# SFR-Vision/6d-pose-estimation

Measured on NVIDIA B200. Metric: ADD-S pose evals/sec (2k-pt mesh), higher is better.
Workload: dtype f32

## Files before the change

### 6d-pose-estimation_b200/csrc/p6d_adds_pruned.cu

```cuda
#include <algorithm>
#include <atomic>
#include <map>
#include <memory>
#include <mutex>
#include <vector>

#include "p6d_common.cuh"

namespace p6d {

constexpr int PR_BLOCK = 32;
constexpr int PR_SUB = 8;
constexpr float PR_SENTINEL = 1.0e18f;
constexpr int PR_MIN_POINTS = 128;

struct PrunedSlot {
    int64_t offset;
    int32_t nb;
    int32_t floats;
};
__host__ __device__ inline int pr_floats(int nb) {
    const int np = PR_BLOCK * nb, nbp = (nb + 3) / 4 * 4;
    return 3 * np + 3 * nbp + 12 * nb + np / 2;
}

struct PrunedTable {
    float* d_sorted = nullptr;
    PrunedSlot* d_slots = nullptr;
    std::vector<PrunedSlot> h_slots;
    int max_nb = 0;
    int max_count = 0;
    std::atomic<bool> enabled{false};
};

static std::mutex g_pr_mu;
static std::map<const p6d_mesh_table*, PrunedTable*> g_pr_tables;

static void kd_split(const float* xyz, std::vector<int>& idx, int lo, int hi) {
    if (hi - lo <= PR_SUB) return;
    const int unit = hi - lo > PR_BLOCK ? PR_BLOCK : PR_SUB;
    float mn[3] = {1e30f, 1e30f, 1e30f}, mx[3] = {-1e30f, -1e30f, -1e30f};
    for (int i = lo; i < hi; ++i)
        for (int c = 0; c < 3; ++c) {
            const float v = xyz[3 * idx[i] + c];
            if (v < mn[c]) mn[c] = v;
            if (v > mx[c]) mx[c] = v;
        }
    int axis = 0;
    for (int c = 1; c < 3; ++c)
        if (mx[c] - mn[c] > mx[axis] - mn[axis]) axis = c;
    const int blocks = (hi - lo + unit - 1) / unit;
    const int mid = lo + (blocks + 1) / 2 * unit;
    auto key = [&](int i) { const float v = xyz[3 * i + axis]; return v == v ? v : 3.0e38f; };
    std::nth_element(idx.begin() + lo, idx.begin() + mid, idx.begin() + hi, [&](int a, int b) {
        const float va = key(a), vb = key(b);
        return va < vb || (va == vb && a < b);
    });
    kd_split(xyz, idx, lo, mid);
    kd_split(xyz, idx, mid, hi);
}

static PrunedTable* build_pruned(const p6d_mesh_table* t, const float* xyz, const int32_t* offsets) {
    std::unique_ptr<PrunedTable> pt(new PrunedTable());
    pt->h_slots.resize(t->n_slots);
    size_t total = 0;
    for (int s = 0; s < t->n_slots; ++s) {
        const int n = t->h_slots[s].count;
        PrunedSlot& ps = pt->h_slots[s];
        ps.nb = (n + PR_BLOCK - 1) / PR_BLOCK;
        ps.floats = pr_floats(ps.nb);
        ps.offset = static_cast<int64_t>(total);
        total += static_cast<size_t>(ps.floats);
        pt->max_nb = std::max(pt->max_nb, ps.nb);
        pt->max_count = std::max(pt->max_count, n);
    }
    std::vector<float> buf(total > 0 ? total : 4, 0.0f);
    for (int s = 0; s < t->n_slots; ++s) {
        const int n = t->h_slots[s].count;
        if (n == 0) continue;
        const PrunedSlot& ps = pt->h_slots[s];
        const float* src = xyz + 3 * static_cast<size_t>(offsets[s]);
        std::vector<int> idx(n);
        for (int i = 0; i < n; ++i) idx[i] = i;
        kd_split(src, idx, 0, n);
        const int np = PR_BLOCK * ps.nb, nbp = (ps.nb + 3) / 4 * 4;
        float* x = buf.data() + ps.offset;
        float* cen = x + 3 * np;
        float* sub = cen + 3 * nbp;
        const int ns = 4 * ps.nb;
        uint16_t* perm = reinterpret_cast<uint16_t*>(sub + 3 * ns);
        for (int b = 0; b < ps.nb; ++b) {
            double c[3] = {0.0, 0.0, 0.0};
            const int cnt = std::min(PR_BLOCK, n - PR_BLOCK * b);
            for (int l = 0; l < PR_BLOCK; ++l) {
                const int p = PR_BLOCK * b + l;
                const int i = idx[l < cnt ? p : PR_BLOCK * b];
                for (int k = 0; k < 3; ++k) x[k * np + p] = src[3 * i + k];
                perm[p] = l < cnt ? static_cast<uint16_t>(i) : 0xffffu;
                if (l < cnt)
                    for (int k = 0; k < 3; ++k) c[k] += src[3 * i + k];
            }
            for (int k = 0; k < 3; ++k) cen[k * nbp + b] = static_cast<float>(c[k] / cnt);
            for (int q = 0; q < PR_BLOCK / PR_SUB; ++q) {
                double sc[3] = {0.0, 0.0, 0.0};
                const int first = PR_BLOCK * b + PR_SUB * q;
                const int scnt = std::max(0, std::min(PR_SUB, n - first));
                for (int l = 0; l < scnt; ++l)
                    for (int k = 0; k < 3; ++k) sc[k] += x[k * np + first + l];
                for (int k = 0; k < 3; ++k)
                    sub[k * ns + 4 * b + q] = scnt > 0 ? static_cast<float>(sc[k] / scnt) : x[k * np + PR_BLOCK * b];
            }
        }
    }
    if (cudaMalloc(&pt->d_sorted, buf.size() * sizeof(float)) != cudaSuccess ||
        cudaMalloc(&pt->d_slots, t->n_slots * sizeof(PrunedSlot)) != cudaSuccess ||
        cudaMemcpy(pt->d_sorted, buf.data(), buf.size() * sizeof(float), cudaMemcpyHostToDevice) != cudaSuccess ||
        cudaMemcpy(pt->d_slots, pt->h_slots.data(), t->n_slots * sizeof(PrunedSlot), cudaMemcpyHostToDevice) !=
            cudaSuccess) {
        cudaGetLastError();
        if (pt->d_sorted) cudaFree(pt->d_sorted);
        if (pt->d_slots) cudaFree(pt->d_slots);
        return nullptr;
    }
    return pt.release();
}

void pruned_table_release(const p6d_mesh_table* t) {
    PrunedTable* pt = nullptr;
    {
        std::lock_guard<std::mutex> lock(g_pr_mu);
        auto it = g_pr_tables.find(t);
        if (it == g_pr_tables.end()) return;
        pt = it->second;
        g_pr_tables.erase(it);
    }
    cudaFree(pt->d_sorted);
    cudaFree(pt->d_slots);
    delete pt;
}

struct PrunedArgs {
    const float* sorted;
    const PrunedSlot* pslots;
};

__host__ __device__ inline size_t pr_smem_floats(int nb, int nmax) {
    const int np = PR_BLOCK * nb;
    return static_cast<size_t>(pr_floats(nb)) + 3 * np + 3 * np + 2 * static_cast<size_t>((nmax + 3) / 4 * 4) + 4 * nb + 16 * nb;
}

__device__ __forceinline__ float eval_block(const float4* __restrict__ q, float px, float py, float pz, float m) {
    float m2 = __int_as_float(0x7f800000);
#pragma unroll
    for (int k = 0; k < PR_BLOCK / 4; ++k) {
        const float4 X = q[3 * k], Y = q[3 * k + 1], Z = q[3 * k + 2];
        const float2 pxx = make_float2(px, px), pyy = make_float2(py, py), pzz = make_float2(pz, pz);
        {
            const float2 dx = sub2(pxx, make_float2(X.x, X.y)), dy = sub2(pyy, make_float2(Y.x, Y.y)),
                         dz = sub2(pzz, make_float2(Z.x, Z.y));
            const float2 s = fma2(dz, dz, fma2(dy, dy, mul2(dx, dx)));
            m = min3_nan(m, s.x, s.y);
        }
        {
            const float2 dx = sub2(pxx, make_float2(X.z, X.w)), dy = sub2(pyy, make_float2(Y.z, Y.w)),
                         dz = sub2(pzz, make_float2(Z.z, Z.w));
            const float2 s = fma2(dz, dz, fma2(dy, dy, mul2(dx, dx)));
            m2 = min3_nan(m2, s.x, s.y);
        }
    }
    return min_nan(m, m2);
}

__device__ __forceinline__ float eval_sub(const float4* __restrict__ q, float px, float py, float pz, float m) {
    const float2 pxx = make_float2(px, px), pyy = make_float2(py, py), pzz = make_float2(pz, pz);
    float m2 = __int_as_float(0x7f800000);
#pragma unroll
    for (int k = 0; k < PR_SUB / 4; ++k) {
        const float4 X = q[3 * k], Y = q[3 * k + 1], Z = q[3 * k + 2];
        {
            const float2 dx = sub2(pxx, make_float2(X.x, X.y)), dy = sub2(pyy, make_float2(Y.x, Y.y)),
                         dz = sub2(pzz, make_float2(Z.x, Z.y));
            const float2 s = fma2(dz, dz, fma2(dy, dy, mul2(dx, dx)));
            m = min3_nan(m, s.x, s.y);
        }
        {
            const float2 dx = sub2(pxx, make_float2(X.z, X.w)), dy = sub2(pyy, make_float2(Y.z, Y.w)),
                         dz = sub2(pzz, make_float2(Z.z, Z.w));
            const float2 s = fma2(dz, dz, fma2(dy, dy, mul2(dx, dx)));
            m2 = min3_nan(m2, s.x, s.y);
        }
    }
    return min_nan(m, m2);
}

__device__ __forceinline__ float eval_two(const float4* __restrict__ q0, const float4* __restrict__ q1, float px, float py,
                                          float pz, float m) {
    const float a = eval_sub(q0, px, py, pz, m);
    const float b = eval_sub(q1, px, py, pz, __int_as_float(0x7f800000));
    return min_nan(a, b);
}

template <int T, int MINB>
__global__ void __launch_bounds__(T, MINB) adds_pruned_kernel(EvalArgs a, PrunedArgs pa, int nb_max, int nmax) {
    constexpr int PR_WARPS = T / 32;
    extern __shared__ __align__(128) unsigned char smem_raw[];
    const int np_max = PR_BLOCK * nb_max;
    float* s_sorted = reinterpret_cast<float*>(smem_raw);
    float* s_gt = s_sorted + pr_floats(nb_max);
    float* s_pred = s_gt + 3 * np_max;
    float* s_dadd = s_pred + 3 * np_max;
    float* s_dadds = s_dadd + (nmax + 3) / 4 * 4;
    float4* s_cp = reinterpret_cast<float4*>(s_dadds + (nmax + 3) / 4 * 4);
    float4* s_cg = s_cp + nb_max;
    __shared__ uint64_t s_bar;
    __shared__ float s_pose[14];
    __shared__ float s_mean[2];
    __shared__ long long s_oid;
    __shared__ int s_next;
    __shared__ int s_blk[2];

    const unsigned full = 0xffffffffu;
    const int tid = threadIdx.x, lane = tid & 31, warp = tid >> 5;
    if (tid == 0) {
        mbar_init(&s_bar, 1);
        fence_mbar_init();
        s_blk[0] = PR_WARPS;
        s_blk[1] = PR_WARPS;
    }
    int par = 0;
    long long staged_oid = -1;
    uint32_t phase = 0;
    if (tid == 0) s_next = atomicAdd(a.work_counter, 1);
    __syncthreads();

    for (;;) {
        const int64_t it = s_next;
        if (it >= a.B) break;
        const int64_t b = a.order ? a.order[it] : it;
        if (tid < 4) s_pose[tid] = __ldg(a.pq + 4 * b + tid);
        else if (tid < 8) s_pose[tid] = __ldg(a.gq + 4 * b + tid - 4);
        else if (tid < 11) s_pose[tid] = __ldg(a.pt + 3 * b + tid - 8);
        else if (tid < 14) s_pose[tid] = __ldg(a.gt + 3 * b + tid - 11);
        else if (tid == 32) s_oid = a.obj[b];
        __syncthreads();
        if (tid == 64) s_next = atomicAdd(a.work_counter, 1);
        const long long oid = s_oid;
        const bool known = oid >= 0 && oid < a.n_slots && a.slots[oid].count > 0;
        if (!known) {
            if (tid == 0) {
                a.add[b] = 0.0f;
                a.adds[b] = 0.0f;
                a.hit[b] = 0;
                a.valid[b] = 0;
                if (a.borderline) a.borderline[b] = 0;
            }
            __syncthreads();
            continue;
        }
        const SlotInfo s = a.slots[oid];
        const PrunedSlot ps = pa.pslots[oid];
        const int n = s.count, nb = ps.nb, np = PR_BLOCK * nb, nbp = (nb + 3) / 4 * 4;
        if (oid != staged_oid) {
            if (tid == 0) {
                fence_proxy_async();
                const uint32_t bytes = static_cast<uint32_t>(ps.floats) * sizeof(float);
                mbar_arrive_expect_tx(&s_bar, bytes);
                tma_bulk_g2s(s_sorted, pa.sorted + ps.offset, bytes, &s_bar);
            }
            mbar_wait(&s_bar, phase);
            phase ^= 1;
            staged_oid = oid;
        }
        const float* mx = s_sorted;
        const float* my = mx + np;
        const float* mz = my + np;
        const float* cen = mz + np;
        const float* sub = cen + 3 * nbp;
        const int ns = 4 * nb;
        const uint16_t* perm = reinterpret_cast<const uint16_t*>(sub + 3 * ns);
        const int mode = s.xform_mode;

        {
            float Rp[9], Rg[9], tp[3], tg[3];
            quat_to_mat(s_pose, Rp);
            quat_to_mat(s_pose + 4, Rg);
#pragma unroll
            for (int k = 0; k < 3; ++k) {
                tp[k] = s_pose[8 + k];
                tg[k] = s_pose[11 + k];
            }
            for (int blk = warp; blk < nb; blk += PR_WARPS) {
                const int p = PR_BLOCK * blk + lane;
                const unsigned orig = perm[p];
                const bool valid = orig != 0xffffu;
                const float x = mx[p], y = my[p], z = mz[p];
                float px, py, pz, qx, qy, qz;
                xform_point(mode, x, y, z, Rp, tp, px, py, pz);
                xform_point(mode, x, y, z, Rg, tg, qx, qy, qz);
                s_pred[p] = px;
                s_pred[np + p] = py;
                s_pred[2 * np + p] = pz;
                float* gq = s_gt + (p >> 2) * 12 + (p & 3);
                gq[0] = valid ? qx : PR_SENTINEL;
                gq[4] = valid ? qy : PR_SENTINEL;
                gq[8] = valid ? qz : PR_SENTINEL;
                if (valid) s_dadd[orig] = __fsqrt_rn(sq3(__fsub_rn(px, qx), __fsub_rn(py, qy), __fsub_rn(pz, qz)));
                const float cx = cen[blk], cy = cen[nbp + blk], cz = cen[2 * nbp + blk];
                const int sb = 4 * blk + (lane >> 3);
                const float sx = sub[sb], sy = sub[ns + sb], sz = sub[2 * ns + sb];
                float cpx, cpy, cpz, cgx, cgy, cgz;
                xform_point(XF_FMA_CHAIN, cx, cy, cz, Rp, tp, cpx, cpy, cpz);
                xform_point(XF_FMA_CHAIN, sx, sy, sz, Rg, tg, cgx, cgy, cgz);
                const float dp = sqrtf(sq3(px - cpx, py - cpy, pz - cpz));
                const float dg = sqrtf(sq3(qx - cgx, qy - cgy, qz - cgz));
                const unsigned rp = __reduce_max_sync(full, valid ? __float_as_uint(dp) : 0u);
                unsigned rg = valid ? __float_as_uint(dg) : 0u;
                rg = max(rg, __shfl_xor_sync(full, rg, 1));
                rg = max(rg, __shfl_xor_sync(full, rg, 2));
                rg = max(rg, __shfl_xor_sync(full, rg, 4));
                if (lane == 0) s_cp[blk] = make_float4(cpx, cpy, cpz, __uint_as_float(rp) * 1.00001f);
                if ((lane & 7) == 0) s_cg[sb] = make_float4(cgx, cgy, cgz, __uint_as_float(rg) * 1.00001f);
            }
        }
        __syncthreads();

        {
            const float4* gq4 = reinterpret_cast<const float4*>(s_gt);
            int A = warp;
            while (A < nb) {
                const int p = PR_BLOCK * A + lane;
                const unsigned orig = perm[p];
                const bool valid = orig != 0xffffu;
                const float px = s_pred[p], py = s_pred[np + p], pz = s_pred[2 * np + p];
                float m = eval_block(gq4 + 24 * A, px, py, pz, __int_as_float(0x7f800000));
                const float4 cA = s_cp[A];
                for (int c0 = 0; c0 < ns; c0 += 32) {
                    const float mmax = __uint_as_float(__reduce_max_sync(full, valid ? __float_as_uint(m) : 0u));
                    const float th = sqrtf(mmax) * 1.0001f + cA.w;
                    const int Bq = c0 + lane;
                    bool cand = false;
                    if (Bq < ns && (Bq >> 2) != A) {
                        const float4 cB = s_cg[Bq];
                        const float dx = cA.x - cB.x, dy = cA.y - cB.y, dz = cA.z - cB.z;
                        const float d2 = dx * dx + dy * dy + dz * dz;
                        const float rhs = th + cB.w;
                        const bool skip = d2 * 0.9999f >= rhs * rhs && d2 < 3.0e38f;
                        cand = !skip;
                    }
                    unsigned todo = __ballot_sync(full, cand);
                    while (todo) {
                        const int b0 = __ffs(todo) - 1;
                        todo &= todo - 1;
                        if (todo) {
                            const int b1 = __ffs(todo) - 1;
                            todo &= todo - 1;
                            m = eval_two(gq4 + 6 * (c0 + b0), gq4 + 6 * (c0 + b1), px, py, pz, m);
                        } else {
                            m = eval_sub(gq4 + 6 * (c0 + b0), px, py, pz, m);
                        }
                    }
                }
                if (valid) s_dadds[orig] = __fsqrt_rn(m);
                int nxt = 0;
                if (lane == 0) nxt = atomicAdd(&s_blk[par], 1);
                A = __shfl_sync(full, nxt, 0);
            }
        }
        __syncthreads();
        if (tid == 0) s_blk[par] = PR_WARPS;
        par ^= 1;

        if (tid < 64) {
            const float* src = tid < 32 ? s_dadd : s_dadds;
            const float mean = aten_mean_warp([&](int e) { return src[e]; }, n, lane);
            if (lane == 0) s_mean[tid >> 5] = mean;
            asm volatile("bar.sync 1, 64;" ::: "memory");
            if (tid == 0) {
                const float add = s_mean[0], adds = s_mean[1];
                const float eff = s.symmetric ? adds : add;
                const bool is_hit = static_cast<double>(eff) < s.threshold;
                a.add[b] = add;
                a.adds[b] = adds;
                a.hit[b] = is_hit ? 1 : 0;
                a.valid[b] = 1;
                if (a.borderline) a.borderline[b] = near_threshold(eff, s.threshold) ? 1 : 0;
                accumulate(a, oid, is_hit, add, adds, true);
            }
        }
    }
}

static size_t g_pr_smem_raised[64];

int launch_eval_pruned(const p6d_mesh_table* table, const EvalArgs& args, cudaStream_t st, bool force, bool* used) {
    *used = false;
    PrunedTable* ptab = nullptr;
    {
        std::lock_guard<std::mutex> lock(g_pr_mu);
        auto it = g_pr_tables.find(table);
        if (it != g_pr_tables.end()) ptab = it->second;
    }
    if (!ptab || (!force && (!ptab->enabled.load(std::memory_order_relaxed) || table->max_count < PR_MIN_POINTS))) return P6D_OK;
    const int nb = ptab->max_nb > 0 ? ptab->max_nb : 1;
    const size_t smem = sizeof(float) * pr_smem_floats(nb, table->max_count);
    {
        std::lock_guard<std::mutex> lock(g_pr_mu);
        size_t& cur = g_pr_smem_raised[table->device & 63];
        if (smem > cur) {
            int limit = 0;
            P6D_CUDA(cudaDeviceGetAttribute(&limit, cudaDevAttrMaxSharedMemoryPerBlockOptin, table->device));
            if (smem + 1024 > static_cast<size_t>(limit)) {
                if (!force) return P6D_OK;
                set_error("largest mesh has %d points; the pruned ADD-S kernel keeps both clouds and the sorted mesh in "
                          "shared memory and accepts at most %d points on this device (p6d_add_eval takes larger meshes)",
                          table->max_count, (limit - 1024) / 4 / 12 / 32 * 32);
                return P6D_ETOOBIG;
            }
            for (const void* fn : {(const void*)adds_pruned_kernel<256, 2>, (const void*)adds_pruned_kernel<256, 3>,
                                   (const void*)adds_pruned_kernel<256, 4>, (const void*)adds_pruned_kernel<128, 8>})
                P6D_CUDA(cudaFuncSetAttribute(fn, cudaFuncAttributeMaxDynamicSharedMemorySize, static_cast<int>(smem)));
            cur = smem;
        }
    }
    EvalArgs a = args;
    a.work_counter = table->d_counters + (__atomic_fetch_add(&table->counter_idx, 1u, __ATOMIC_RELAXED) % P6D_NUM_COUNTERS);
    P6D_CUDA(cudaMemsetAsync(a.work_counter, 0, sizeof(int), st));
    struct Shape { const void* fn; int threads, minb; };
    const Shape shapes[] = {{(const void*)adds_pruned_kernel<128, 8>, 128, 8}, {(const void*)adds_pruned_kernel<256, 4>, 256, 4},
                            {(const void*)adds_pruned_kernel<256, 3>, 256, 3}, {(const void*)adds_pruned_kernel<256, 2>, 256, 2}};
    const Shape* pick = &shapes[3];
    int per_sm = 0;
    for (const Shape& sh : shapes) {
        if (sh.threads == 128 && nb > 16) continue;
        int occ = 0;
        P6D_CUDA(cudaOccupancyMaxActiveBlocksPerMultiprocessor(&occ, sh.fn, sh.threads, smem));
        if (occ >= sh.minb || &sh == &shapes[3]) {
            pick = &sh;
            per_sm = occ;
            break;
        }
    }
    if (per_sm < 1) per_sm = 1;
    int64_t grid = static_cast<int64_t>(table->sm_count) * per_sm;
    if (grid > a.B) grid = a.B;
    PrunedArgs pa{ptab->d_sorted, ptab->d_slots};
    int nb_arg = nb, nmax_arg = table->max_count;
    void* kargs[] = {&a, &pa, &nb_arg, &nmax_arg};
    P6D_CUDA(cudaLaunchKernel(pick->fn, dim3(static_cast<unsigned>(grid)), dim3(pick->threads), kargs, smem, st));
    P6D_CUDA(cudaGetLastError());
    *used = true;
    return P6D_OK;
}

}

using namespace p6d;

extern "C" {

void p6d_internal_build_pruned(const p6d_mesh_table* t, const float* xyz, const int32_t* offsets) {
    if (t->max_count > 65534) return;
    PrunedTable* pt = nullptr;
    try {
        pt = build_pruned(t, xyz, offsets);
    } catch (...) {
        return;
    }
    if (!pt) return;
    std::lock_guard<std::mutex> lock(g_pr_mu);
    g_pr_tables[t] = pt;
}

void p6d_internal_release_pruned(const p6d_mesh_table* t) { pruned_table_release(t); }

int p6d_mesh_table_set_pruning(p6d_mesh_table* table, int enable) {
    if (!table) { set_error("p6d_mesh_table_set_pruning: table is NULL"); return P6D_EINVAL; }
    std::lock_guard<std::mutex> lock(g_pr_mu);
    auto it = g_pr_tables.find(table);
    if (it == g_pr_tables.end()) {
        if (!enable) return P6D_OK;
        set_error("p6d_mesh_table_set_pruning: this table has no block structure (a mesh with more than 65,534 points, "
                  "or out of memory at creation)");
        return P6D_ETOOBIG;
    }
    it->second->enabled.store(enable != 0, std::memory_order_relaxed);
    return P6D_OK;
}

int p6d_add_eval_pruned(const p6d_mesh_table* table, const float* pq, const float* pt, const float* gq,
                        const float* gt, const int64_t* obj, const int32_t* order, int64_t B, float* add,
                        float* adds, uint8_t* hit, uint8_t* valid, uint8_t* borderline,
                        const p6d_accumulators* acc, void* stream) {
    if (!table || B < 0 || (B > 0 && (!pq || !pt || !gq || !gt || !obj || !add || !adds || !hit || !valid))) {
        set_error("p6d_add_eval_pruned: bad arguments");
        return P6D_EINVAL;
    }
    auto mis = [](const void* p, size_t al) { return p && (reinterpret_cast<uintptr_t>(p) & (al - 1)) != 0; };
    if (mis(pq, 4) || mis(pt, 4) || mis(gq, 4) || mis(gt, 4) || mis(obj, 8) || mis(order, 4) || mis(add, 4) || mis(adds, 4)) {
        set_error("p6d_add_eval_pruned: a pointer is not aligned to its element size");
        return P6D_EINVAL;
    }
    if (B == 0) return P6D_OK;
    if (B > static_cast<int64_t>(INT32_MAX) - (1 << 20)) {
        set_error("p6d_add_eval_pruned: B = %lld exceeds the per-launch limit of %d poses; split the batch",
                  static_cast<long long>(B), INT32_MAX - (1 << 20));
        return P6D_EINVAL;
    }
    DeviceGuard guard(table->device);
    if (!guard.ok) return cuda_fail(cudaGetLastError(), "cudaSetDevice");
    EvalArgs a{};
    fill_eval_args(table, a);
    a.pq = pq; a.pt = pt; a.gq = gq; a.gt = gt; a.obj = obj; a.order = order; a.B = B;
    a.add = add; a.adds = adds; a.hit = hit; a.valid = valid; a.borderline = borderline;
    if (acc) { a.acc = *acc; a.has_acc = 1; }
    bool used = false;
    const int rc = launch_eval_pruned(table, a, static_cast<cudaStream_t>(stream), true, &used);
    if (rc == P6D_OK && !used) {
        set_error("p6d_add_eval_pruned: this table has no block structure (a mesh with more than 65,534 points, or out of "
                  "memory at creation)");
        return P6D_ETOOBIG;
    }
    return rc;
}

}
```

Before: 1.386 million.

## Read sorted mesh from global, drop pred smem, prune with per-sub-block spheres

```diff
diff --git a/6d-pose-estimation_b200/csrc/p6d_adds_pruned.cu b/6d-pose-estimation_b200/csrc/p6d_adds_pruned.cu
--- a/6d-pose-estimation_b200/csrc/p6d_adds_pruned.cu
+++ b/6d-pose-estimation_b200/csrc/p6d_adds_pruned.cu
@@ -19,9 +19,9 @@
     int32_t nb;
     int32_t floats;
 };
-__host__ __device__ inline int pr_floats(int nb) {
-    const int np = PR_BLOCK * nb, nbp = (nb + 3) / 4 * 4;
-    return 3 * np + 3 * nbp + 12 * nb + np / 2;
+inline int pr_floats(int nb) {
+    const int np = PR_BLOCK * nb;
+    return 3 * np + 12 * nb + np / 2;
 }
 
 struct PrunedTable {
@@ -83,24 +83,19 @@
         std::vector<int> idx(n);
         for (int i = 0; i < n; ++i) idx[i] = i;
         kd_split(src, idx, 0, n);
-        const int np = PR_BLOCK * ps.nb, nbp = (ps.nb + 3) / 4 * 4;
+        const int np = PR_BLOCK * ps.nb;
         float* x = buf.data() + ps.offset;
-        float* cen = x + 3 * np;
-        float* sub = cen + 3 * nbp;
+        float* sub = x + 3 * np;
         const int ns = 4 * ps.nb;
         uint16_t* perm = reinterpret_cast<uint16_t*>(sub + 3 * ns);
         for (int b = 0; b < ps.nb; ++b) {
-            double c[3] = {0.0, 0.0, 0.0};
             const int cnt = std::min(PR_BLOCK, n - PR_BLOCK * b);
             for (int l = 0; l < PR_BLOCK; ++l) {
                 const int p = PR_BLOCK * b + l;
                 const int i = idx[l < cnt ? p : PR_BLOCK * b];
                 for (int k = 0; k < 3; ++k) x[k * np + p] = src[3 * i + k];
                 perm[p] = l < cnt ? static_cast<uint16_t>(i) : 0xffffu;
-                if (l < cnt)
-                    for (int k = 0; k < 3; ++k) c[k] += src[3 * i + k];
-            }
-            for (int k = 0; k < 3; ++k) cen[k * nbp + b] = static_cast<float>(c[k] / cnt);
+            }
             for (int q = 0; q < PR_BLOCK / PR_SUB; ++q) {
                 double sc[3] = {0.0, 0.0, 0.0};
                 const int first = PR_BLOCK * b + PR_SUB * q;
@@ -146,7 +141,7 @@
 
 __host__ __device__ inline size_t pr_smem_floats(int nb, int nmax) {
     const int np = PR_BLOCK * nb;
-    return static_cast<size_t>(pr_floats(nb)) + 3 * np + 3 * np + 2 * static_cast<size_t>((nmax + 3) / 4 * 4) + 4 * nb + 16 * nb;
+    return 3 * static_cast<size_t>(np) + 2 * static_cast<size_t>((nmax + 3) / 4 * 4) + 32 * static_cast<size_t>(nb);
 }
 
 __device__ __forceinline__ float eval_block(const float4* __restrict__ q, float px, float py, float pz, float m) {
@@ -200,19 +195,20 @@
     return min_nan(a, b);
 }
 
+#ifdef P6D_DEV
+__device__ unsigned long long g_pr_sub_evals;
+#endif
+
 template <int T, int MINB>
 __global__ void __launch_bounds__(T, MINB) adds_pruned_kernel(EvalArgs a, PrunedArgs pa, int nb_max, int nmax) {
     constexpr int PR_WARPS = T / 32;
     extern __shared__ __align__(128) unsigned char smem_raw[];
     const int np_max = PR_BLOCK * nb_max;
-    float* s_sorted = reinterpret_cast<float*>(smem_raw);
-    float* s_gt = s_sorted + pr_floats(nb_max);
-    float* s_pred = s_gt + 3 * np_max;
-    float* s_dadd = s_pred + 3 * np_max;
+    float4* s_cp = reinterpret_cast<float4*>(smem_raw);
+    float4* s_cg = s_cp + 4 * nb_max;
+    float* s_gt = reinterpret_cast<float*>(s_cg + 4 * nb_max);
+    float* s_dadd = s_gt + 3 * np_max;
     float* s_dadds = s_dadd + (nmax + 3) / 4 * 4;
-    float4* s_cp = reinterpret_cast<float4*>(s_dadds + (nmax + 3) / 4 * 4);
-    float4* s_cg = s_cp + nb_max;
-    __shared__ uint64_t s_bar;
     __shared__ float s_pose[14];
     __shared__ float s_mean[2];
     __shared__ long long s_oid;
@@ -222,14 +218,10 @@
     const unsigned full = 0xffffffffu;
     const int tid = threadIdx.x, lane = tid & 31, warp = tid >> 5;
     if (tid == 0) {
-        mbar_init(&s_bar, 1);
-        fence_mbar_init();
         s_blk[0] = PR_WARPS;
         s_blk[1] = PR_WARPS;
     }
     int par = 0;
-    long long staged_oid = -1;
-    uint32_t phase = 0;
     if (tid == 0) s_next = atomicAdd(a.work_counter, 1);
     __syncthreads();
 
@@ -259,24 +251,11 @@
         }
         const SlotInfo s = a.slots[oid];
         const PrunedSlot ps = pa.pslots[oid];
-        const int n = s.count, nb = ps.nb, np = PR_BLOCK * nb, nbp = (nb + 3) / 4 * 4;
-        if (oid != staged_oid) {
-            if (tid == 0) {
-                fence_proxy_async();
-                const uint32_t bytes = static_cast<uint32_t>(ps.floats) * sizeof(float);
-                mbar_arrive_expect_tx(&s_bar, bytes);
-                tma_bulk_g2s(s_sorted, pa.sorted + ps.offset, bytes, &s_bar);
-            }
-            mbar_wait(&s_bar, phase);
-            phase ^= 1;
-            staged_oid = oid;
-        }
-        const float* mx = s_sorted;
+        const int n = s.count, nb = ps.nb, np = PR_BLOCK * nb, ns = 4 * nb;
+        const float* mx = pa.sorted + ps.offset;
         const float* my = mx + np;
         const float* mz = my + np;
-        const float* cen = mz + np;
-        const float* sub = cen + 3 * nbp;
-        const int ns = 4 * nb;
+        const float* sub = mz + np;
         const uint16_t* perm = reinterpret_cast<const uint16_t*>(sub + 3 * ns);
         const int mode = s.xform_mode;
 
@@ -291,63 +270,88 @@
             }
             for (int blk = warp; blk < nb; blk += PR_WARPS) {
                 const int p = PR_BLOCK * blk + lane;
-                const unsigned orig = perm[p];
+                const unsigned orig = __ldg(perm + p);
                 const bool valid = orig != 0xffffu;
-                const float x = mx[p], y = my[p], z = mz[p];
+                const float x = __ldg(mx + p), y = __ldg(my + p), z = __ldg(mz + p);
                 float px, py, pz, qx, qy, qz;
                 xform_point(mode, x, y, z, Rp, tp, px, py, pz);
                 xform_point(mode, x, y, z, Rg, tg, qx, qy, qz);
-                s_pred[p] = px;
-                s_pred[np + p] = py;
-                s_pred[2 * np + p] = pz;
                 float* gq = s_gt + (p >> 2) * 12 + (p & 3);
                 gq[0] = valid ? qx : PR_SENTINEL;
                 gq[4] = valid ? qy : PR_SENTINEL;
                 gq[8] = valid ? qz : PR_SENTINEL;
                 if (valid) s_dadd[orig] = __fsqrt_rn(sq3(__fsub_rn(px, qx), __fsub_rn(py, qy), __fsub_rn(pz, qz)));
-                const float cx = cen[blk], cy = cen[nbp + blk], cz = cen[2 * nbp + blk];
                 const int sb = 4 * blk + (lane >> 3);
-                const float sx = sub[sb], sy = sub[ns + sb], sz = sub[2 * ns + sb];
+                const float sx = __ldg(sub + sb), sy = __ldg(sub + ns + sb), sz = __ldg(sub + 2 * ns + sb);
                 float cpx, cpy, cpz, cgx, cgy, cgz;
-                xform_point(XF_FMA_CHAIN, cx, cy, cz, Rp, tp, cpx, cpy, cpz);
+                xform_point(XF_FMA_CHAIN, sx, sy, sz, Rp, tp, cpx, cpy, cpz);
                 xform_point(XF_FMA_CHAIN, sx, sy, sz, Rg, tg, cgx, cgy, cgz);
                 const float dp = sqrtf(sq3(px - cpx, py - cpy, pz - cpz));
                 const float dg = sqrtf(sq3(qx - cgx, qy - cgy, qz - cgz));
-                const unsigned rp = __reduce_max_sync(full, valid ? __float_as_uint(dp) : 0u);
+                unsigned rp = valid ? __float_as_uint(dp) : 0u;
                 unsigned rg = valid ? __float_as_uint(dg) : 0u;
-                rg = max(rg, __shfl_xor_sync(full, rg, 1));
-                rg = max(rg, __shfl_xor_sync(full, rg, 2));
-                rg = max(rg, __shfl_xor_sync(full, rg, 4));
-                if (lane == 0) s_cp[blk] = make_float4(cpx, cpy, cpz, __uint_as_float(rp) * 1.00001f);
-                if ((lane & 7) == 0) s_cg[sb] = make_float4(cgx, cgy, cgz, __uint_as_float(rg) * 1.00001f);
+#pragma unroll
+                for (int o = 1; o < PR_SUB; o <<= 1) {
+                    rp = max(rp, __shfl_xor_sync(full, rp, o));
+                    rg = max(rg, __shfl_xor_sync(full, rg, o));
+                }
+                if ((lane & 7) == 0) {
+                    s_cp[sb] = make_float4(cpx, cpy, cpz, __uint_as_float(rp) * 1.00001f);
+                    s_cg[sb] = make_float4(cgx, cgy, cgz, __uint_as_float(rg) * 1.00001f);
+                }
             }
         }
         __syncthreads();
 
         {
             const float4* gq4 = reinterpret_cast<const float4*>(s_gt);
+#ifdef P6D_DEV
+            unsigned evals = 0;
+#endif
             int A = warp;
             while (A < nb) {
                 const int p = PR_BLOCK * A + lane;
-                const unsigned orig = perm[p];
+                const unsigned orig = __ldg(perm + p);
                 const bool valid = orig != 0xffffu;
-                const float px = s_pred[p], py = s_pred[np + p], pz = s_pred[2 * np + p];
+                float px, py, pz;
+                {
+                    float Rp[9], tp[3];
+                    quat_to_mat(s_pose, Rp);
+#pragma unroll
+                    for (int k = 0; k < 3; ++k) tp[k] = s_pose[8 + k];
+                    xform_point(mode, __ldg(mx + p), __ldg(my + p), __ldg(mz + p), Rp, tp, px, py, pz);
+                }
                 float m = eval_block(gq4 + 24 * A, px, py, pz, __int_as_float(0x7f800000));
-                const float4 cA = s_cp[A];
+                const float4* cP = s_cp + 4 * A;
+#ifdef P6D_DEV
+                evals += PR_BLOCK / PR_SUB;
+#endif
                 for (int c0 = 0; c0 < ns; c0 += 32) {
-                    const float mmax = __uint_as_float(__reduce_max_sync(full, valid ? __float_as_uint(m) : 0u));
-                    const float th = sqrtf(mmax) * 1.0001f + cA.w;
+                    unsigned mm = valid ? __float_as_uint(m) : 0u;
+#pragma unroll
+                    for (int o = 1; o < PR_SUB; o <<= 1) mm = max(mm, __shfl_xor_sync(full, mm, o));
+                    const float thl = sqrtf(__uint_as_float(mm)) * 1.0001f + cP[lane >> 3].w;
+                    float th[PR_BLOCK / PR_SUB];
+#pragma unroll
+                    for (int k = 0; k < PR_BLOCK / PR_SUB; ++k) th[k] = __shfl_sync(full, thl, PR_SUB * k);
                     const int Bq = c0 + lane;
                     bool cand = false;
                     if (Bq < ns && (Bq >> 2) != A) {
                         const float4 cB = s_cg[Bq];
-                        const float dx = cA.x - cB.x, dy = cA.y - cB.y, dz = cA.z - cB.z;
-                        const float d2 = dx * dx + dy * dy + dz * dz;
-                        const float rhs = th + cB.w;
-                        const bool skip = d2 * 0.9999f >= rhs * rhs && d2 < 3.0e38f;
-                        cand = !skip;
+#pragma unroll
+                        for (int k = 0; k < PR_BLOCK / PR_SUB; ++k) {
+                            const float4 c = cP[k];
+                            const float dx = c.x - cB.x, dy = c.y - cB.y, dz = c.z - cB.z;
+                            const float d2 = dx * dx + dy * dy + dz * dz;
+                            const float rhs = th[k] + cB.w;
+                            const bool skip = d2 * 0.9999f >= rhs * rhs && d2 < 3.0e38f;
+                            cand |= !skip;
+                        }
                     }
                     unsigned todo = __ballot_sync(full, cand);
+#ifdef P6D_DEV
+                    evals += __popc(todo);
+#endif
                     while (todo) {
                         const int b0 = __ffs(todo) - 1;
                         todo &= todo - 1;
@@ -365,6 +369,9 @@
                 if (lane == 0) nxt = atomicAdd(&s_blk[par], 1);
                 A = __shfl_sync(full, nxt, 0);
             }
+#ifdef P6D_DEV
+            if (lane == 0 && evals) atomicAdd(&g_pr_sub_evals, static_cast<unsigned long long>(evals));
+#endif
         }
         __syncthreads();
         if (tid == 0) s_blk[par] = PR_WARPS;
@@ -407,13 +414,18 @@
         std::lock_guard<std::mutex> lock(g_pr_mu);
         size_t& cur = g_pr_smem_raised[table->device & 63];
         if (smem > cur) {
-            int limit = 0;
-            P6D_CUDA(cudaDeviceGetAttribute(&limit, cudaDevAttrMaxSharedMemoryPerBlockOptin, table->device));
-            if (smem + 1024 > static_cast<size_t>(limit)) {
+            int per_sm = 0, reserved = 0;
+            cudaFuncAttributes fa{};
+            P6D_CUDA(cudaDeviceGetAttribute(&per_sm, cudaDevAttrMaxSharedMemoryPerMultiprocessor, table->device));
+            P6D_CUDA(cudaDeviceGetAttribute(&reserved, cudaDevAttrReservedSharedMemoryPerBlock, table->device));
+            P6D_CUDA(cudaFuncGetAttributes(&fa, (const void*)adds_pruned_kernel<256, 2>));
+            const size_t fit = static_cast<size_t>(per_sm / 2 - reserved) - fa.sharedSizeBytes;
+            if (smem > fit) {
                 if (!force) return P6D_OK;
-                set_error("largest mesh has %d points; the pruned ADD-S kernel keeps both clouds and the sorted mesh in "
-                          "shared memory and accepts at most %d points on this device (p6d_add_eval takes larger meshes)",
-                          table->max_count, (limit - 1024) / 4 / 12 / 32 * 32);
+                set_error("largest mesh has %d points; the pruned ADD-S kernel keeps the gt cloud, both distance rows and "
+                          "the bounding spheres in shared memory (24 bytes per point), needs two CTAs per SM and accepts "
+                          "at most %d points on this device (p6d_add_eval takes larger meshes)",
+                          table->max_count, static_cast<int>(fit / 24 / 32 * 32));
                 return P6D_ETOOBIG;
             }
             for (const void* fn : {(const void*)adds_pruned_kernel<256, 2>, (const void*)adds_pruned_kernel<256, 3>,
@@ -523,4 +535,15 @@
     return rc;
 }
 
-}
+#ifdef P6D_DEV
+__attribute__((visibility("default"))) int p6d_dev_pruned_sub_evals(int reset, unsigned long long* out) {
+    if (out) P6D_CUDA(cudaMemcpyFromSymbol(out, g_pr_sub_evals, sizeof(unsigned long long)));
+    if (reset) {
+        const unsigned long long zero = 0;
+        P6D_CUDA(cudaMemcpyToSymbol(g_pr_sub_evals, &zero, sizeof(zero)));
+    }
+    return P6D_OK;
+}
+#endif
+
+}
```

Result: no change. 1.386 million (median of 6 runs) (-0.0%).
